# HagenMarin/SHAP-Transformer-ASR

Hardware: NVIDIA B200
Metric: masked_coalition_forwards_per_sec (higher is better)
Workload: dtype bf16

## Files before the change

### shap_transformer_asr_b200/csrc/common.cuh

```cuda
#pragma once
#include <cuda_runtime.h>
#include <cuda_bf16.h>
#include <cuda.h>
#include <stdint.h>
#include <string>

namespace w2s {

#define W2S_CUDA_OK(expr)                                                                        \
  do {                                                                                           \
    cudaError_t _e = (expr);                                                                     \
    if (_e != cudaSuccess) {                                                                     \
      return std::string(#expr) + ": " + cudaGetErrorString(_e) + " (" __FILE__ ":" +          \
             std::to_string(__LINE__) + ")";                                                     \
    }                                                                                            \
  } while (0)

}
#include <cstdlib>
#include <utility>
namespace w2s {
template <typename... KArgs, typename... Args>
inline cudaError_t launch_pdl(void (*kernel)(KArgs...), dim3 grid, dim3 block, size_t smem, cudaStream_t s, int cluster_x,
                              Args&&... args) {
// ... 178 lines not shown
      "cp.async.bulk.tensor.4d.shared::cluster.global.mbarrier::complete_tx::bytes [%0], [%1, {%3, %4, %5, %6}], [%2];"
      ::"r"(dst), "l"(reinterpret_cast<uint64_t>(map)), "r"(bar), "r"(c0), "r"(c1), "r"(c2), "r"(c3)
      : "memory");
}
__device__ __forceinline__ void tma_load_3d_mc(uint32_t dst, const CUtensorMap* map, uint32_t bar, int c0, int c1,
                                               int c2, uint16_t cta_mask) {
  asm volatile(
      "cp.async.bulk.tensor.3d.shared::cluster.global.mbarrier::complete_tx::bytes.multicast::cluster"
      " [%0], [%1, {%3, %4, %5}], [%2], %6;"
      ::"r"(dst), "l"(reinterpret_cast<uint64_t>(map)), "r"(bar), "r"(c0), "r"(c1), "r"(c2), "h"(cta_mask)
      : "memory");
}
__device__ __forceinline__ uint32_t cluster_ctarank() {
  uint32_t r;
  asm volatile("mov.u32 %0, %%cluster_ctarank;" : "=r"(r));
  return r;
}
__device__ __forceinline__ uint32_t mapa_u32(uint32_t local_addr, uint32_t rank) {
  uint32_t r;
  asm volatile("mapa.shared::cluster.u32 %0, %1, %2;" : "=r"(r) : "r"(local_addr), "r"(rank));
  return r;
}
__device__ __forceinline__ void mbar_arrive_cluster(uint32_t cluster_addr) {
  asm volatile("mbarrier.arrive.shared::cluster.b64 _, [%0];" ::"r"(cluster_addr) : "memory");
}
__device__ __forceinline__ void tma_load_3d_2sm(uint32_t dst, const CUtensorMap* map, uint32_t bar_cluster, int c0,
                                                int c1, int c2) {
  asm volatile(
      "cp.async.bulk.tensor.3d.cta_group::2.shared::cluster.global.mbarrier::complete_tx::bytes"
      " [%0], [%1, {%3, %4, %5}], [%2];"
      ::"r"(dst), "l"(reinterpret_cast<uint64_t>(map)), "r"(bar_cluster), "r"(c0), "r"(c1), "r"(c2)
      : "memory");
}
__device__ __forceinline__ void tma_load_4d_2sm(uint32_t dst, const CUtensorMap* map, uint32_t bar_cluster, int c0,
                                                int c1, int c2, int c3) {
  asm volatile(
      "cp.async.bulk.tensor.4d.cta_group::2.shared::cluster.global.mbarrier::complete_tx::bytes"
      " [%0], [%1, {%3, %4, %5, %6}], [%2];"
      ::"r"(dst), "l"(reinterpret_cast<uint64_t>(map)), "r"(bar_cluster), "r"(c0), "r"(c1), "r"(c2), "r"(c3)
      : "memory");
}
template <int kCols>
__device__ __forceinline__ void tmem_alloc_2sm(uint32_t smem_dst) {
  asm volatile("tcgen05.alloc.cta_group::2.sync.aligned.shared::cta.b32 [%0], %1;" ::"r"(smem_dst), "n"(kCols)
               : "memory");
}
__device__ __forceinline__ void tmem_relinquish_2sm() {
  asm volatile("tcgen05.relinquish_alloc_permit.cta_group::2.sync.aligned;" ::: "memory");
}
template <int kCols>
__device__ __forceinline__ void tmem_dealloc_2sm(uint32_t taddr) {
  asm volatile("tcgen05.dealloc.cta_group::2.sync.aligned.b32 %0, %1;" ::"r"(taddr), "n"(kCols) : "memory");
}
__device__ __forceinline__ void umma_bf16_2sm(uint32_t tmem_d, uint64_t desc_a, uint64_t desc_b, uint32_t idesc,
                                              uint32_t accumulate) {
  asm volatile(
      "{\n\t.reg .pred p;\n\t"
      "setp.ne.b32 p, %4, 0;\n\t"
      "tcgen05.mma.cta_group::2.kind::f16 [%0], %1, %2, %3, p;\n\t}"
      ::"r"(tmem_d), "l"(desc_a), "l"(desc_b), "r"(idesc), "r"(accumulate)
      : "memory");
}
__device__ __forceinline__ void umma_commit_2sm_mc(uint32_t bar, uint16_t cta_mask) {
  asm volatile(
      "tcgen05.commit.cta_group::2.mbarrier::arrive::one.shared::cluster.multicast::cluster.b64 [%0], %1;"
      ::"r"(bar), "h"(cta_mask)
      : "memory");
}
__device__ __forceinline__ void cluster_sync_all() {
  asm volatile("barrier.cluster.arrive.release.aligned;" ::: "memory");
  asm volatile("barrier.cluster.wait.acquire.aligned;" ::: "memory");
}
__device__ __forceinline__ void tma_store_4d(const CUtensorMap* map, uint32_t src, int c0, int c1, int c2, int c3) {
  asm volatile("cp.async.bulk.tensor.4d.global.shared::cta.bulk_group [%0, {%2, %3, %4, %5}], [%1];"
               ::"l"(reinterpret_cast<uint64_t>(map)), "r"(src), "r"(c0), "r"(c1), "r"(c2), "r"(c3)
               : "memory");
}
__device__ __forceinline__ void tma_reduce_add_4d(const CUtensorMap* map, uint32_t src, int c0, int c1, int c2, int c3) {
  asm volatile("cp.reduce.async.bulk.tensor.4d.global.shared::cta.add.tile.bulk_group [%0, {%2, %3, %4, %5}], [%1];"
               ::"l"(reinterpret_cast<uint64_t>(map)), "r"(src), "r"(c0), "r"(c1), "r"(c2), "r"(c3)
               : "memory");
}
__device__ __forceinline__ void tma_store_commit() { asm volatile("cp.async.bulk.commit_group;" ::: "memory"); }
__device__ __forceinline__ void tma_store_wait_read() { asm volatile("cp.async.bulk.wait_group.read 0;" ::: "memory"); }
__device__ __forceinline__ void tma_store_wait_all() { asm volatile("cp.async.bulk.wait_group 0;" ::: "memory"); }
__device__ __forceinline__ void sts128(uint32_t addr, uint32_t a, uint32_t b, uint32_t c, uint32_t d) {
  asm volatile("st.shared.v4.b32 [%0], {%1, %2, %3, %4};" ::"r"(addr), "r"(a), "r"(b), "r"(c), "r"(d) : "memory");
}
__device__ __forceinline__ void tma_prefetch_l2_4d(const CUtensorMap* map, int c0, int c1, int c2, int c3) {
  asm volatile("cp.async.bulk.prefetch.tensor.4d.L2.global.tile [%0, {%1, %2, %3, %4}];"
               ::"l"(reinterpret_cast<uint64_t>(map)), "r"(c0), "r"(c1), "r"(c2), "r"(c3)
               : "memory");
}
__device__ __forceinline__ void tma_prefetch_desc(const CUtensorMap* map) {
  asm volatile("prefetch.tensormap [%0];" ::"l"(reinterpret_cast<uint64_t>(map)) : "memory");
}

template <int kCols>
__device__ __forceinline__ void tmem_alloc(uint32_t smem_dst) {
  asm volatile("tcgen05.alloc.cta_group::1.sync.aligned.shared::cta.b32 [%0], %1;" ::"r"(smem_dst), "n"(kCols)
               : "memory");
}
__device__ __forceinline__ void tmem_relinquish() {
  asm volatile("tcgen05.relinquish_alloc_permit.cta_group::1.sync.aligned;" ::: "memory");
}
template <int kCols>
__device__ __forceinline__ void tmem_dealloc(uint32_t taddr) {
  asm volatile("tcgen05.dealloc.cta_group::1.sync.aligned.b32 %0, %1;" ::"r"(taddr), "n"(kCols) : "memory");
}
__device__ __forceinline__ void tc_fence_before() {
  asm volatile("tcgen05.fence::before_thread_sync;" ::: "memory");
}
__device__ __forceinline__ void tc_fence_after() {
  asm volatile("tcgen05.fence::after_thread_sync;" ::: "memory");
}
__device__ __forceinline__ void umma_bf16(uint32_t tmem_d, uint64_t desc_a, uint64_t desc_b, uint32_t idesc,
                                          uint32_t accumulate) {
  asm volatile(
      "{\n\t.reg .pred p;\n\t"
      "setp.ne.b32 p, %4, 0;\n\t"
      "tcgen05.mma.cta_group::1.kind::f16 [%0], %1, %2, %3, p;\n\t}"
      ::"r"(tmem_d), "l"(desc_a), "l"(desc_b), "r"(idesc), "r"(accumulate)
      : "memory");
}
__device__ __forceinline__ bool elect_one() {
  uint32_t pred;
  asm volatile(
      "{\n\t.reg .pred p;\n\t"
      "elect.sync _|p, 0xffffffff;\n\t"
      "selp.u32 %0, 1, 0, p;\n\t}"
      : "=r"(pred));
  return pred != 0;
}
__device__ __forceinline__ void umma_commit(uint32_t bar) {
  asm volatile("tcgen05.commit.cta_group::1.mbarrier::arrive::one.shared::cluster.b64 [%0];" ::"r"(bar)
               : "memory");
}
__device__ __forceinline__ void umma_commit_mc(uint32_t bar, uint16_t cta_mask) {
  asm volatile(
      "tcgen05.commit.cta_group::1.mbarrier::arrive::one.shared::cluster.multicast::cluster.b64 [%0], %1;"
      ::"r"(bar), "h"(cta_mask)
      : "memory");
}
__device__ __forceinline__ void tmem_ld_wait() { asm volatile("tcgen05.wait::ld.sync.aligned;" ::: "memory"); }

__device__ __forceinline__ void tmem_ld_32x32(uint32_t taddr, float (&v)[32]) {
  uint32_t r[32];
  asm volatile(
      "tcgen05.ld.sync.aligned.32x32b.x32.b32 "
      "{%0, %1, %2, %3, %4, %5, %6, %7, %8, %9, %10, %11, %12, %13, %14, %15, "
      "%16, %17, %18, %19, %20, %21, %22, %23, %24, %25, %26, %27, %28, %29, %30, %31}, [%32];"
      : "=r"(r[0]), "=r"(r[1]), "=r"(r[2]), "=r"(r[3]), "=r"(r[4]), "=r"(r[5]), "=r"(r[6]), "=r"(r[7]),
        "=r"(r[8]), "=r"(r[9]), "=r"(r[10]), "=r"(r[11]), "=r"(r[12]), "=r"(r[13]), "=r"(r[14]), "=r"(r[15]),
        "=r"(r[16]), "=r"(r[17]), "=r"(r[18]), "=r"(r[19]), "=r"(r[20]), "=r"(r[21]), "=r"(r[22]), "=r"(r[23]),
        "=r"(r[24]), "=r"(r[25]), "=r"(r[26]), "=r"(r[27]), "=r"(r[28]), "=r"(r[29]), "=r"(r[30]), "=r"(r[31])
      : "r"(taddr)
      : "memory");
  tmem_ld_wait();
#pragma unroll
  for (int i = 0; i < 32; ++i) v[i] = __uint_as_float(r[i]);
}
__device__ __forceinline__ void tmem_ld_32x32_issue(uint32_t taddr, float (&v)[32]) {
  asm volatile(
      "tcgen05.ld.sync.aligned.32x32b.x32.b32 "
      "{%0, %1, %2, %3, %4, %5, %6, %7, %8, %9, %10, %11, %12, %13, %14, %15, "
      "%16, %17, %18, %19, %20, %21, %22, %23, %24, %25, %26, %27, %28, %29, %30, %31}, [%32];"
      : "=f"(v[0]), "=f"(v[1]), "=f"(v[2]), "=f"(v[3]), "=f"(v[4]), "=f"(v[5]), "=f"(v[6]), "=f"(v[7]),
// ... 36 lines not shown
```

### shap_transformer_asr_b200/csrc/gemm.cu

```cuda
#include "gemm.cuh"
#include "gemm_epi.cuh"

#include <cudaTypedefs.h>
#include <cstdlib>
#include <mutex>

namespace w2s {

template <int BN>
struct TcCfg {
  static constexpr int BM = 128, BK = 64;
  static constexpr int A_BYTES = BM * BK * 2;
  static constexpr int B_BYTES = BN * BK * 2;
  static constexpr int STAGE_BYTES = A_BYTES + B_BYTES;
  static constexpr int STAGES = BN >= 256 ? 4 : (BN >= 128 ? 6 : 8);
  static constexpr int ACC_COLS = BN <= 32 ? 32 : (BN <= 64 ? 64 : (BN <= 128 ? 128 : 256));
  static constexpr int TMEM_COLS = 2 * ACC_COLS;
  static constexpr int CH = (BN % 32 == 0) ? 32 : 16;
  static constexpr size_t SMEM = (size_t)STAGES * STAGE_BYTES + 1024 + 256;
};

struct TileCoord {
  int g, b, m0, n0;
};
// ... 152 lines not shown
  const int nt = tile % tiles_n;
  tile /= tiles_n;
  const int mt = tile % tiles_m;
  tile /= tiles_m;
  const int b = tile % p.Bz, g = tile / p.Bz;
  const int m0 = mt * 64, n0 = nt * 64;
  const int tx = threadIdx.x & 15, ty = threadIdx.x >> 4;
  float acc[4][4] = {};
  const int rowlen = p.a_kb_per_row * 64;
  for (int k0 = 0; k0 < p.K; k0 += 16) {
    for (int i = threadIdx.x; i < 64 * 16; i += 256) {
      const int r = i >> 4, kk = i & 15;
      const int k = k0 + kk;
      float av = 0.f, wv = 0.f;
      if (k < p.K) {
        const long long row = (long long)g * p.a_g_row + m0 + r + k / rowlen;
        const long long col = (long long)g * p.a_g_col + k % rowlen;
        if (row < p.a_rows && col < p.a_cols)
          av = __bfloat162float(p.a[(long long)b * p.a_batch_stride + row * p.a_row_stride + col]);
        if (n0 + r < p.N) wv = __bfloat162float(p.w[((long long)g * p.N + n0 + r) * p.K + k]);
      }
      As[kk][r] = av;
      Ws[kk][r] = wv;
    }
    __syncthreads();
#pragma unroll
    for (int kk = 0; kk < 16; ++kk) {
      float a[4], w[4];
#pragma unroll
      for (int i = 0; i < 4; ++i) {
        a[i] = As[kk][ty * 4 + i];
        w[i] = Ws[kk][tx * 4 + i];
      }
#pragma unroll
      for (int i = 0; i < 4; ++i)
#pragma unroll
        for (int j = 0; j < 4; ++j) acc[i][j] = fmaf(a[i], w[j], acc[i][j]);
    }
    __syncthreads();
  }
#pragma unroll
  for (int i = 0; i < 4; ++i) {
    const int m = m0 + ty * 4 + i;
    if (m < p.M) epi_store<4>(p.epi, p.N, g, b, m, n0 + tx * 4, acc[i]);
  }
}

static PFN_cuTensorMapEncodeTiled_v12000 g_encode = nullptr;
static std::once_flag g_init_once;
static std::string g_init_err;

template <int BN>
static cudaError_t set_attr() {
  return cudaFuncSetAttribute(gemm_tc_kernel<BN>, cudaFuncAttributeMaxDynamicSharedMemorySize, (int)TcCfg<BN>::SMEM);
}

std::string gemm_init() {
  std::call_once(g_init_once, [] {
    void* fn = nullptr;
    cudaDriverEntryPointQueryResult qres;
    cudaError_t e = cudaGetDriverEntryPoint("cuTensorMapEncodeTiled", &fn, cudaEnableDefault, &qres);
    if (e != cudaSuccess || qres != cudaDriverEntryPointSuccess || fn == nullptr) {
      g_init_err = "cuTensorMapEncodeTiled entry point not available (driver too old?)";
      return;
    }
    g_encode = reinterpret_cast<PFN_cuTensorMapEncodeTiled_v12000>(fn);
    cudaError_t a = set_attr<256>();
    if (a == cudaSuccess) a = set_attr<128>();
    if (a == cudaSuccess) a = set_attr<64>();
    if (a == cudaSuccess) a = set_attr<48>();
    if (a == cudaSuccess) a = set_attr<32>();
    if (a != cudaSuccess) g_init_err = std::string("cudaFuncSetAttribute(gemm_tc_kernel): ") + cudaGetErrorString(a);
    if (g_init_err.empty()) g_init_err = gemm2_init();
  });
  return g_init_err;
}

std::string make_tensor_map_bf16(CUtensorMap* map, const void* base, int rank, const uint64_t* dims,
                                 const uint64_t* strides_bytes, const uint32_t* box) {
  return make_tensor_map(map, base, 0, rank, dims, strides_bytes, box);
}

std::string make_tensor_map(CUtensorMap* map, const void* base, int fp32, int rank, const uint64_t* dims,
                            const uint64_t* strides_bytes, const uint32_t* box) {
  if (!g_encode) return "tensor map encoder not initialised";
  cuuint64_t gdim[5];
  cuuint64_t gstr[5];
  cuuint32_t bx[5];
  cuuint32_t es[5];
  for (int i = 0; i < rank; ++i) {
    gdim[i] = dims[i];
    bx[i] = box[i];
    es[i] = 1;
  }
  for (int i = 0; i + 1 < rank; ++i) gstr[i] = strides_bytes[i];
  CUresult r = g_encode(map, fp32 ? CU_TENSOR_MAP_DATA_TYPE_FLOAT32 : CU_TENSOR_MAP_DATA_TYPE_BFLOAT16, rank, const_cast<void*>(base), gdim, gstr, bx, es,
                        CU_TENSOR_MAP_INTERLEAVE_NONE, CU_TENSOR_MAP_SWIZZLE_128B,
                        CU_TENSOR_MAP_L2_PROMOTION_L2_256B, CU_TENSOR_MAP_FLOAT_OOB_FILL_NONE);
  if (r != CUDA_SUCCESS) {
    std::string s = "cuTensorMapEncodeTiled failed (CUresult " + std::to_string((int)r) + ") rank=" +
                    std::to_string(rank) + " dims=";
    for (int i = 0; i < rank; ++i) s += std::to_string(dims[i]) + ",";
    s += " strides=";
    for (int i = 0; i + 1 < rank; ++i) s += std::to_string(strides_bytes[i]) + ",";
    return s;
  }
  return "";
}

static int pick_bn(int N) {
  if (N % 256 == 0) return 256;
  if (N % 128 == 0) return 128;
  if (N % 64 == 0) return 64;
  if (N % 48 == 0) return 48;
  if (N % 32 == 0) return 32;
  return 0;
}

std::string gemm_prepare(const GemmProblem& p, int num_sms, GemmLaunch* out) {
  if (p.K % 64 != 0) return "gemm: K must be a multiple of 64 (got " + std::to_string(p.K) + ")";
  const int bn = pick_bn(p.N);
  if (bn == 0) return "gemm: N must be a multiple of 32 or 48 (got " + std::to_string(p.N) + ")";
  if (p.epi.glu && (bn % 32 != 0)) return "gemm: GLU epilogue needs N % 32 == 0";
  GemmDev& d = out->dev;
  d.M = p.M; d.N = p.N; d.K = p.K; d.Bz = p.Bz; d.G = p.G;
  d.tiles_m = (p.M + 127) / 128;
  d.tiles_n = p.N / bn;
  d.num_tiles = d.tiles_m * d.tiles_n * p.Bz * p.G;
  d.num_kb = p.K / 64;
  out->mc = (bn >= 128 && d.tiles_m >= 2 && d.num_tiles >= num_sms) ? 2 : 0;
  d.units_m = out->mc ? (d.tiles_m + 1) / 2 : d.tiles_m;
  d.num_units = d.units_m * d.tiles_n * p.Bz * p.G;
  d.a_kb_per_row = p.a_kb_per_row;
  d.a_g_col = p.a_g_col;
  d.a_g_row = p.a_g_row;
  d.w_batched = p.w_batch_stride != 0;
  d.a = p.a; d.w = p.w;
  d.a_cols = p.a_cols; d.a_rows = p.a_rows; d.a_row_stride = p.a_row_stride; d.a_batch_stride = p.a_batch_stride;
  d.epi = p.epi;
  out->bn = bn;
  if (out->mc) {
    const int clusters = d.num_units < num_sms / 2 ? d.num_units : num_sms / 2;
    out->grid = 2 * clusters;
  } else {
    out->grid = d.num_units < num_sms ? d.num_units : num_sms;
  }
  out->smem = bn == 256 ? TcCfg<256>::SMEM : bn == 128 ? TcCfg<128>::SMEM : bn == 64 ? TcCfg<64>::SMEM
              : bn == 48 ? TcCfg<48>::SMEM : TcCfg<32>::SMEM;
  if ((p.a_row_stride * 2) % 16 || (p.a_batch_stride * 2) % 16 || (reinterpret_cast<uintptr_t>(p.a) % 16))
    return "gemm: A view must be 16-byte aligned in base and strides";
  {
    uint64_t dims[3] = {(uint64_t)p.a_cols, (uint64_t)p.a_rows, (uint64_t)p.a_batches};
    uint64_t str[2] = {(uint64_t)p.a_row_stride * 2, (uint64_t)(p.a_batches > 1 ? p.a_batch_stride : p.a_row_stride * p.a_rows) * 2};
    uint32_t box[3] = {64, 128, 1};
    W2S_TRY(make_tensor_map_bf16(&out->mapA, p.a, 3, dims, str, box));
  }
  {
    const uint64_t rs = (uint64_t)(p.w_row_stride ? p.w_row_stride : p.K);
    const uint64_t wr = (uint64_t)(p.w_rows ? p.w_rows : p.N);
    const uint64_t gs = (uint64_t)(p.w_g_stride ? p.w_g_stride : (long long)p.K * p.N);
    const uint64_t bs = p.w_batch_stride ? (uint64_t)p.w_batch_stride : gs * (uint64_t)p.G;
    uint64_t dims[4] = {(uint64_t)p.K, wr, (uint64_t)p.G, (uint64_t)(p.w_batch_stride ? p.Bz : 1)};
    uint64_t str[3] = {rs * 2, gs * 2, bs * 2};
    uint32_t box[4] = {64, (uint32_t)(out->mc ? bn / 2 : bn), 1, 1};
    W2S_TRY(make_tensor_map_bf16(&out->mapW, p.w, 4, dims, str, box));
  }
  out->tma_out = 0;
  if (out->mc == 2 && !p.epi.glu) {
    const uint64_t es = p.epi.out_fp32 ? 4 : 2;
    const uint64_t ldb = p.Bz > 1 ? (uint64_t)p.epi.ldb : (uint64_t)p.epi.ldm * p.M;
    const uint64_t ldg = p.G > 1 ? (uint64_t)p.epi.ldg : ldb * p.Bz;
    uint64_t dims[4] = {(uint64_t)p.N, (uint64_t)p.M, (uint64_t)p.Bz, (uint64_t)p.G};
    uint64_t str[3] = {(uint64_t)p.epi.ldm * es, ldb * es, ldg * es};
    uint32_t box[4] = {p.epi.out_fp32 ? 32u : 64u, 32, 1, 1};
    if (str[0] % 16 == 0 && str[1] % 16 == 0 && str[2] % 16 == 0 && reinterpret_cast<uintptr_t>(p.epi.out) % 16 == 0) {
      W2S_TRY(make_tensor_map(&out->mapOut, p.epi.out, p.epi.out_fp32, 4, dims, str, box));
      out->tma_out = 1;
    }
  }
  return "";
}

std::string gemm_launch_tc(const GemmLaunch& l, cudaStream_t s) {
  if (l.mc == 2) return gemm2_launch(l, s);
  switch (l.bn) {
    case 256: W2S_CUDA_OK(launch_pdl(gemm_tc_kernel<256>, dim3(l.grid), dim3(384), l.smem, s, 1, l.mapA, l.mapW, l.dev)); break;
    case 128: W2S_CUDA_OK(launch_pdl(gemm_tc_kernel<128>, dim3(l.grid), dim3(384), l.smem, s, 1, l.mapA, l.mapW, l.dev)); break;
    case 64: W2S_CUDA_OK(launch_pdl(gemm_tc_kernel<64>, dim3(l.grid), dim3(384), l.smem, s, 1, l.mapA, l.mapW, l.dev)); break;
    case 48: W2S_CUDA_OK(launch_pdl(gemm_tc_kernel<48>, dim3(l.grid), dim3(384), l.smem, s, 1, l.mapA, l.mapW, l.dev)); break;
    case 32: W2S_CUDA_OK(launch_pdl(gemm_tc_kernel<32>, dim3(l.grid), dim3(384), l.smem, s, 1, l.mapA, l.mapW, l.dev)); break;
    default: return "gemm: bad BN";
  }
  W2S_CUDA_OK(cudaGetLastError());
  return "";
}

std::string gemm_launch_simt(const GemmLaunch& l, cudaStream_t s) {
  const GemmDev& d = l.dev;
  const long long tiles = (long long)((d.M + 63) / 64) * ((d.N + 63) / 64) * d.Bz * d.G;
  gemm_simt_kernel<<<(unsigned)tiles, 256, 0, s>>>(d);
  W2S_CUDA_OK(cudaGetLastError());
  return "";
}

}
```

### shap_transformer_asr_b200/csrc/gemm.cuh

```cuda
#pragma once
#include "common.cuh"

namespace w2s {

struct EpiParams {
  const float* bias = nullptr;
  int act = ACT_NONE;
  int glu = 0;
  float alpha = 1.0f;
  const void* residual = nullptr;
  int res_fp32 = 0;
  void* out = nullptr;
  int out_fp32 = 0;
  long long ldg = 0, ldb = 0, ldm = 0;
};

struct GemmProblem {
  const __nv_bfloat16* a = nullptr;
  long long a_cols = 0, a_rows = 0, a_batches = 1;
  long long a_row_stride = 0, a_batch_stride = 0;
  int a_kb_per_row = 1, a_g_col = 0, a_g_row = 0;
  const __nv_bfloat16* w = nullptr;
  long long w_row_stride = 0, w_g_stride = 0, w_batch_stride = 0;
  int w_rows = 0;
  int M = 0, N = 0, K = 0, Bz = 1, G = 1;
  EpiParams epi;
};

struct GemmDev {
  int M, N, K, Bz, G;
  int tiles_m, tiles_n, num_tiles, num_kb;
  int units_m, num_units;
  int a_kb_per_row, a_g_col, a_g_row;
  int w_batched;
  const __nv_bfloat16* a;
  const __nv_bfloat16* w;
  long long a_cols, a_rows, a_row_stride, a_batch_stride;
  EpiParams epi;
};

struct GemmLaunch {
  CUtensorMap mapA, mapW;
  CUtensorMap mapOut;
  int tma_out = 0;
  GemmDev dev;
  int bn = 0;
  int mc = 0;
  int grid = 0;
  size_t smem = 0;
};

std::string gemm_prepare(const GemmProblem& p, int num_sms, GemmLaunch* out);
std::string gemm_launch_tc(const GemmLaunch& l, cudaStream_t s);
std::string gemm_launch_simt(const GemmLaunch& l, cudaStream_t s);
std::string gemm2_init();
std::string gemm2_launch(const GemmLaunch& l, cudaStream_t s);
std::string gemm_init();

std::string make_tensor_map_bf16(CUtensorMap* map, const void* base, int rank, const uint64_t* dims,
                                 const uint64_t* strides_bytes, const uint32_t* box);
std::string make_tensor_map(CUtensorMap* map, const void* base, int fp32, int rank, const uint64_t* dims,
                            const uint64_t* strides_bytes, const uint32_t* box);

}
```

### shap_transformer_asr_b200/csrc/gemm2.cu

```cuda
#include "gemm.cuh"
#include "gemm_epi.cuh"

namespace w2s {

template <int BN>
struct Tc2Cfg {
  static constexpr int A_BYTES = 128 * 64 * 2;
  static constexpr int B_BYTES = (BN / 2) * 64 * 2;
  static constexpr int STAGE_BYTES = A_BYTES + B_BYTES;
  static constexpr int EPI_BYTES = 8 * 4096 + 8 * 512;
  static constexpr int STAGES = (227 * 1024 - 1024 - 256 - EPI_BYTES) / STAGE_BYTES > 8
                                    ? 8 : (227 * 1024 - 1024 - 256 - EPI_BYTES) / STAGE_BYTES;
  static constexpr int ACC_COLS = BN;
  static constexpr int TMEM_COLS = 2 * ACC_COLS;
  static constexpr size_t SMEM = (size_t)STAGES * STAGE_BYTES + EPI_BYTES + 1024 + 256;
};

template <int BN>
__global__ void __launch_bounds__(384, 1)
gemm_tc2_kernel(const __grid_constant__ CUtensorMap mapA, const __grid_constant__ CUtensorMap mapW,
                const __grid_constant__ CUtensorMap mapOut, const GemmDev p, const int tma_out) {
  using C = Tc2Cfg<BN>;
  const uint32_t rank = cluster_ctarank();
  const bool leader = rank == 0;
  const int unit0 = (int)(blockIdx.x >> 1), unit_step = (int)(gridDim.x >> 1);
  extern __shared__ uint8_t smem_raw[];
  const uint32_t raw = smem_u32(smem_raw);
  const uint32_t tiles = (raw + 1023u) & ~1023u;
  uint8_t* tiles_ptr = smem_raw + (tiles - raw);
  const uint32_t epi_smem = tiles + C::STAGES * C::STAGE_BYTES;
  const uint32_t bars = epi_smem + C::EPI_BYTES;
  auto full_bar = [&](int s) { return bars + 8u * s; };
  auto empty_bar = [&](int s) { return bars + 8u * (C::STAGES + s); };
  auto tfull_bar = [&](int a) { return bars + 8u * (2 * C::STAGES + a); };
  auto tempty_bar = [&](int a) { return bars + 8u * (2 * C::STAGES + 2 + a); };
  const uint32_t tmem_slot = bars + 8u * (2 * C::STAGES + 4);
  volatile uint32_t* tmem_slot_ptr =
      reinterpret_cast<volatile uint32_t*>(tiles_ptr + C::STAGES * C::STAGE_BYTES + C::EPI_BYTES + 8 * (2 * C::STAGES + 4));

  const int warp = threadIdx.x >> 5, lane = threadIdx.x & 31;
  if (warp == 8 && lane == 0) {
    tma_prefetch_desc(&mapA);
    tma_prefetch_desc(&mapW);
    if (tma_out) tma_prefetch_desc(&mapOut);
  }
  if (warp == 9 && lane == 0) {
    for (int s = 0; s < C::STAGES; ++s) {
      mbar_init(full_bar(s), 1);
      mbar_init(empty_bar(s), 1);
    }
    for (int a = 0; a < 2; ++a) {
      mbar_init(tfull_bar(a), 1);
      mbar_init(tempty_bar(a), 16);
    }
    fence_barrier_init();
    fence_proxy_async();
  }
  if (warp == 10) {
    tmem_alloc_2sm<C::TMEM_COLS>(tmem_slot);
    tmem_relinquish_2sm();
  }
  tc_fence_before();
  __syncthreads();
  cluster_sync_all();
  tc_fence_after();
  const uint32_t tmem_base = *tmem_slot_ptr;

  if (warp == 8) {
    if (elect_one()) {
      int stage = 0;
      uint32_t phase = 0;
      for (int unit = unit0; unit < p.num_units; unit += unit_step) {
        int nt = unit % p.tiles_n;
        int r = unit / p.tiles_n;
        const int mu = r % p.units_m;
        r /= p.units_m;
        const int b = r % p.Bz, g = r / p.Bz;
        const int m0 = (2 * mu + (int)rank) * 128, n0 = nt * BN;
        for (int kb = 0; kb < p.num_kb; ++kb) {
          mbar_wait(empty_bar(stage), phase ^ 1u);
          const uint32_t full_leader = mapa_u32(full_bar(stage), 0);
          if (leader) mbar_expect_tx(full_bar(stage), 2 * C::STAGE_BYTES);
          const int krow = kb / p.a_kb_per_row;
          const int kcol = kb - krow * p.a_kb_per_row;
          const uint32_t sa = tiles + stage * C::STAGE_BYTES;
          tma_load_3d_2sm(sa, &mapA, full_leader, g * p.a_g_col + kcol * 64, g * p.a_g_row + m0 + krow, b);
          tma_load_4d_2sm(sa + C::A_BYTES, &mapW, full_leader, kb * 64, n0 + (int)rank * (BN / 2), g, p.w_batched ? b : 0);
          if (++stage == C::STAGES) {
            stage = 0;
            phase ^= 1u;
          }
        }
      }
    }
  } else if (warp == 9) {
    if (leader && elect_one()) {
      constexpr uint32_t idesc = umma_idesc_bf16(256, BN);
      int stage = 0;
      uint32_t phase = 0;
      int acc = 0;
      uint32_t acc_phase = 0;
      for (int unit = unit0; unit < p.num_units; unit += unit_step) {
        mbar_wait(tempty_bar(acc), acc_phase ^ 1u);
        tc_fence_after();
        const uint32_t d_tmem = tmem_base + acc * C::ACC_COLS;
        for (int kb = 0; kb < p.num_kb; ++kb) {
          mbar_wait(full_bar(stage), phase);
          tc_fence_after();
          const uint32_t sa = tiles + stage * C::STAGE_BYTES;
          const uint64_t da = umma_desc_sw128(sa);
          const uint64_t db = umma_desc_sw128(sa + C::A_BYTES);
#pragma unroll
          for (int k = 0; k < 4; ++k) umma_bf16_2sm(d_tmem, da + 2u * k, db + 2u * k, idesc, (kb | k) != 0 ? 1u : 0u);
          umma_commit_2sm_mc(empty_bar(stage), (uint16_t)0x3);
          if (++stage == C::STAGES) {
            stage = 0;
            phase ^= 1u;
          }
        }
        umma_commit_2sm_mc(tfull_bar(acc), (uint16_t)0x3);
        acc ^= 1;
        if (acc == 0) acc_phase ^= 1u;
      }
    }
  } else if (warp < 8) {
    const int q = warp & 3, hsel = warp >> 2;
    const bool lead = elect_one();
    const uint32_t stg = epi_smem + warp * 4096;
    const uint32_t stg_row = stg + lane * 128;
    float* sbias = reinterpret_cast<float*>(tiles_ptr + C::STAGES * C::STAGE_BYTES + 8 * 4096 + warp * 512);
    const bool f32 = p.epi.out_fp32 != 0;
    const bool reduce_add = tma_out && f32 && p.epi.res_fp32 && p.epi.residual == p.epi.out;
    int acc = 0;
    uint32_t acc_phase = 0;
    for (int unit = unit0; unit < p.num_units; unit += unit_step) {
      int nt = unit % p.tiles_n;
      int r = unit / p.tiles_n;
      const int mu = r % p.units_m;
      r /= p.units_m;
      const int b = r % p.Bz, g = r / p.Bz;
      const int m0 = (2 * mu + (int)rank) * 128, n0 = nt * BN;
      const int m = m0 + q * 32 + lane;
      const bool row_ok = m < p.M;
      const uint32_t t0 = tmem_base + (static_cast<uint32_t>(q * 32) << 16) + acc * C::ACC_COLS;
      if (tma_out) {
        const int bw = f32 ? 32 : 64;
        const int nblk = BN / (2 * bw);
        if (p.epi.bias) {
          for (int i = lane; i < nblk * bw; i += 32) {
            const int col = (2 * (i / bw) + hsel) * bw + (i % bw);
            sbias[i] = __ldg(p.epi.bias + (long long)g * p.N + n0 + col);
          }
        }
        __syncwarp();
        mbar_wait(tfull_bar(acc), acc_phase);
        tc_fence_after();
        const int nsub = f32 ? nblk : 2 * nblk;
        auto sub_col = [&](int sidx) { return f32 ? (2 * sidx + hsel) * 32 : (2 * (sidx >> 1) + hsel) * 64 + (sidx & 1) * 32; };
        float v[32];
        tmem_ld_32x32_issue(t0 + sub_col(0), v);
#pragma unroll 1
        for (int sidx = 0; sidx < nsub; ++sidx) {
          const int c = sub_col(sidx);
          const int sub = f32 ? 0 : (sidx & 1);
          tmem_ld_wait();
          epi_math32(p.epi, p.epi.bias ? sbias + sidx * 32 : nullptr, p.N, g, b, m, n0 + c, row_ok, v, reduce_add);
          if (f32) {
            if (lead) tma_store_wait_read();
            __syncwarp();
#pragma unroll
            for (int j = 0; j < 8; ++j)
              sts128(stg_row + (((uint32_t)j ^ ((uint32_t)lane & 7u)) << 4), __float_as_uint(v[4 * j]),
                     __float_as_uint(v[4 * j + 1]), __float_as_uint(v[4 * j + 2]), __float_as_uint(v[4 * j + 3]));
            if (sidx + 1 < nsub) tmem_ld_32x32_issue(t0 + sub_col(sidx + 1), v);
          } else {
            uint32_t pk[16];
#pragma unroll
            for (int j = 0; j < 16; ++j) pk[j] = pack_bf16x2(v[2 * j], v[2 * j + 1]);
            if (sidx + 1 < nsub) tmem_ld_32x32_issue(t0 + sub_col(sidx + 1), v);
            if (sub == 0) {
              if (lead) tma_store_wait_read();
              __syncwarp();
            }
#pragma unroll
            for (int j = 0; j < 4; ++j)
              sts128(stg_row + (((uint32_t)(sub * 4 + j) ^ ((uint32_t)lane & 7u)) << 4), pk[4 * j], pk[4 * j + 1],
                     pk[4 * j + 2], pk[4 * j + 3]);
          }
          if (f32 || sub == 1) {
            const int cblk = f32 ? c : c - 32;
            fence_proxy_async();
            __syncwarp();
            if (lead) {
              if (reduce_add) tma_reduce_add_4d(&mapOut, stg, n0 + cblk, m0 + q * 32, b, g);
              else tma_store_4d(&mapOut, stg, n0 + cblk, m0 + q * 32, b, g);
              tma_store_commit();
            }
          }
        }
      } else {
        mbar_wait(tfull_bar(acc), acc_phase);
        tc_fence_after();
#pragma unroll 1
        for (int c = hsel * 32; c < BN; c += 64) {
          float v[32];
          tmem_ld_32x32(t0 + c, v);
          if (row_ok) epi_store<32>(p.epi, p.N, g, b, m, n0 + c, v);
        }
      }
      tc_fence_before();
      __syncwarp();
      if (lane == 0) {
        if (leader) mbar_arrive(tempty_bar(acc));
        else mbar_arrive_cluster(mapa_u32(tempty_bar(acc), 0));
      }
      acc ^= 1;
      if (acc == 0) acc_phase ^= 1u;
    }
    if (tma_out && lead) tma_store_wait_all();
  }

  tc_fence_before();
  __syncthreads();
  cluster_sync_all();
  if (warp == 10) {
    tc_fence_after();
    tmem_dealloc_2sm<C::TMEM_COLS>(tmem_base);
  }
}

std::string gemm2_init() {
  cudaError_t e = cudaFuncSetAttribute(gemm_tc2_kernel<256>, cudaFuncAttributeMaxDynamicSharedMemorySize,
                                       (int)Tc2Cfg<256>::SMEM);
  if (e == cudaSuccess)
    e = cudaFuncSetAttribute(gemm_tc2_kernel<128>, cudaFuncAttributeMaxDynamicSharedMemorySize, (int)Tc2Cfg<128>::SMEM);
  if (e != cudaSuccess) return std::string("cudaFuncSetAttribute(gemm_tc2_kernel): ") + cudaGetErrorString(e);
  return "";
}

size_t gemm2_smem(int bn) { return bn == 256 ? Tc2Cfg<256>::SMEM : Tc2Cfg<128>::SMEM; }

template <int BN>
static cudaError_t launch2(const GemmLaunch& l, cudaStream_t s) {
  return launch_pdl(gemm_tc2_kernel<BN>, dim3(l.grid), dim3(384), Tc2Cfg<BN>::SMEM, s, 2, l.mapA, l.mapW,
                    l.tma_out ? l.mapOut : l.mapA, l.dev, l.tma_out);
}

std::string gemm2_launch(const GemmLaunch& l, cudaStream_t s) {
  if (l.bn == 256) W2S_CUDA_OK(launch2<256>(l, s));
  else if (l.bn == 128) W2S_CUDA_OK(launch2<128>(l, s));
  else return "gemm (CTA pair): BN must be 256 or 128";
  return "";
}

}
```

### shap_transformer_asr_b200/csrc/gemm_epi.cuh

```cuda
#pragma once
#include "gemm.cuh"

namespace w2s {

template <int CH>
__device__ __forceinline__ void epi_store(const EpiParams& e, int N, int g, int b, int m, int ncol0, float* v) {
  if (ncol0 >= N) return;
  if (e.bias) {
    const float4* bp = reinterpret_cast<const float4*>(e.bias + (long long)g * N + ncol0);
#pragma unroll
    for (int j = 0; j < CH / 4; ++j) {
      const float4 t = __ldg(bp + j);
      v[4 * j] += t.x;
      v[4 * j + 1] += t.y;
      v[4 * j + 2] += t.z;
      v[4 * j + 3] += t.w;
    }
  }
  if (e.act == ACT_GELU) {
#pragma unroll
    for (int j = 0; j < CH; j += 2) {
      const float2 r = gelu_erf2(make_float2(v[j], v[j + 1]));
      v[j] = r.x;
      v[j + 1] = r.y;
    }
  } else if (e.act == ACT_SWISH) {
#pragma unroll
    for (int j = 0; j < CH; ++j) v[j] = swish(v[j]);
  }
  int nout0 = ncol0, nvals = CH, Nout = N;
  if (e.glu) {
#pragma unroll
    for (int j = 0; j < CH / 2; ++j) v[j] = v[2 * j] * rcp_approx(1.0f + ex2_approx(-1.4426950408889634f * v[2 * j + 1]));
    nout0 = ncol0 >> 1;
    nvals = CH / 2;
    Nout = N >> 1;
  }
  const long long off = (long long)g * e.ldg + (long long)b * e.ldb + (long long)m * e.ldm + nout0;
  if constexpr (CH < 8) {
#pragma unroll
    for (int j = 0; j < CH; ++j) {
      if (j < nvals && nout0 + j < Nout) {
        float r = 0.f;
        if (e.residual)
          r = e.res_fp32 ? reinterpret_cast<const float*>(e.residual)[off + j]
                         : __bfloat162float(reinterpret_cast<const __nv_bfloat16*>(e.residual)[off + j]);
        const float o = fmaf(v[j], e.alpha, r);
        if (e.out_fp32) reinterpret_cast<float*>(e.out)[off + j] = o;
        else reinterpret_cast<__nv_bfloat16*>(e.out)[off + j] = __float2bfloat16_rn(o);
      }
    }
  } else {
    if (e.residual) {
      if (e.res_fp32) {
        const float* rp = reinterpret_cast<const float*>(e.residual) + off;
#pragma unroll
        for (int j = 0; j < CH; j += 4) {
          if (j < nvals && nout0 + j < Nout) {
            float4 r = *reinterpret_cast<const float4*>(rp + j);
            v[j] = fmaf(v[j], e.alpha, r.x);
            v[j + 1] = fmaf(v[j + 1], e.alpha, r.y);
            v[j + 2] = fmaf(v[j + 2], e.alpha, r.z);
            v[j + 3] = fmaf(v[j + 3], e.alpha, r.w);
          }
        }
      } else {
        const __nv_bfloat16* rp = reinterpret_cast<const __nv_bfloat16*>(e.residual) + off;
#pragma unroll
        for (int j = 0; j < CH; j += 4) {
          if (j < nvals && nout0 + j < Nout) {
            uint2 r = *reinterpret_cast<const uint2*>(rp + j);
            v[j] = fmaf(v[j], e.alpha, bf16_lo(r.x));
            v[j + 1] = fmaf(v[j + 1], e.alpha, bf16_hi(r.x));
            v[j + 2] = fmaf(v[j + 2], e.alpha, bf16_lo(r.y));
            v[j + 3] = fmaf(v[j + 3], e.alpha, bf16_hi(r.y));
          }
        }
      }
    } else if (e.alpha != 1.0f) {
#pragma unroll
      for (int j = 0; j < CH; ++j) v[j] *= e.alpha;
    }
    if (e.out_fp32) {
      float* op = reinterpret_cast<float*>(e.out) + off;
#pragma unroll
      for (int j = 0; j < CH; j += 4)
        if (j < nvals && nout0 + j < Nout)
          *reinterpret_cast<float4*>(op + j) = make_float4(v[j], v[j + 1], v[j + 2], v[j + 3]);
    } else {
      __nv_bfloat16* op = reinterpret_cast<__nv_bfloat16*>(e.out) + off;
#pragma unroll
      for (int j = 0; j < CH; j += 8) {
        if (j < nvals && nout0 + j < Nout) {
          uint4 u;
          u.x = pack_bf16x2(v[j], v[j + 1]);
          u.y = pack_bf16x2(v[j + 2], v[j + 3]);
          u.z = pack_bf16x2(v[j + 4], v[j + 5]);
          u.w = pack_bf16x2(v[j + 6], v[j + 7]);
          *reinterpret_cast<uint4*>(op + j) = u;
        }
      }
    }
  }
}


__device__ __forceinline__ void epi_math32(const EpiParams& e, const float* sbias, int N, int g, int b, int m,
                                           int ncol0, bool row_ok, float* v, bool skip_residual = false) {
  if (sbias) {
#pragma unroll
    for (int j = 0; j < 8; ++j) {
      const float4 t = *reinterpret_cast<const float4*>(sbias + 4 * j);
      v[4 * j] += t.x;
      v[4 * j + 1] += t.y;
      v[4 * j + 2] += t.z;
      v[4 * j + 3] += t.w;
    }
  }
  if (e.act == ACT_GELU) {
#pragma unroll
    for (int j = 0; j < 32; j += 2) {
      const float2 r = gelu_erf2(make_float2(v[j], v[j + 1]));
      v[j] = r.x;
      v[j + 1] = r.y;
    }
  } else if (e.act == ACT_SWISH) {
#pragma unroll
    for (int j = 0; j < 32; ++j) v[j] = swish(v[j]);
  }
  if (e.residual && !skip_residual) {
    if (row_ok) {
      const long long off = (long long)g * e.ldg + (long long)b * e.ldb + (long long)m * e.ldm + ncol0;
      if (e.res_fp32) {
        const float* rp = reinterpret_cast<const float*>(e.residual) + off;
#pragma unroll
        for (int j = 0; j < 32; j += 4) {
          const float4 r = *reinterpret_cast<const float4*>(rp + j);
          v[j] = fmaf(v[j], e.alpha, r.x);
          v[j + 1] = fmaf(v[j + 1], e.alpha, r.y);
          v[j + 2] = fmaf(v[j + 2], e.alpha, r.z);
          v[j + 3] = fmaf(v[j + 3], e.alpha, r.w);
        }
      } else {
        const __nv_bfloat16* rp = reinterpret_cast<const __nv_bfloat16*>(e.residual) + off;
#pragma unroll
        for (int j = 0; j < 32; j += 8) {
          const uint4 r = *reinterpret_cast<const uint4*>(rp + j);
          v[j] = fmaf(v[j], e.alpha, bf16_lo(r.x));
          v[j + 1] = fmaf(v[j + 1], e.alpha, bf16_hi(r.x));
          v[j + 2] = fmaf(v[j + 2], e.alpha, bf16_lo(r.y));
          v[j + 3] = fmaf(v[j + 3], e.alpha, bf16_hi(r.y));
          v[j + 4] = fmaf(v[j + 4], e.alpha, bf16_lo(r.z));
          v[j + 5] = fmaf(v[j + 5], e.alpha, bf16_hi(r.z));
          v[j + 6] = fmaf(v[j + 6], e.alpha, bf16_lo(r.w));
          v[j + 7] = fmaf(v[j + 7], e.alpha, bf16_hi(r.w));
        }
      }
    }
  } else if (e.alpha != 1.0f) {
#pragma unroll
    for (int j = 0; j < 32; ++j) v[j] *= e.alpha;
  }
}

}
```

Measured before the change: 12490.

## Restructure CTA-pair GEMM epilogue with 16 warps, smaller swizzled TMA boxes, early TMEM release

Templates the pair GEMM kernel on the number of epilogue warps and picks 16 epilogue warps for activation-heavy, short-K GEMMs. Output TMA stores now use 32-column (bf16) or 16-column (fp32) boxes with 64B swizzle, and several store buffers are kept in flight by waiting on all but the newest groups. Bias for the next tile is prefetched into registers, and the accumulator is released to the MMA warp before the final epilogue math runs. The aim is to hide epilogue cost behind the mainloop; the risks are more TMA store instructions, higher register pressure and a more complex sync pattern.

```diff
diff --git a/shap_transformer_asr_b200/csrc/common.cuh b/shap_transformer_asr_b200/csrc/common.cuh
--- a/shap_transformer_asr_b200/csrc/common.cuh
+++ b/shap_transformer_asr_b200/csrc/common.cuh
@@ -284,7 +284,10 @@
                : "memory");
 }
 __device__ __forceinline__ void tma_store_commit() { asm volatile("cp.async.bulk.commit_group;" ::: "memory"); }
-__device__ __forceinline__ void tma_store_wait_read() { asm volatile("cp.async.bulk.wait_group.read 0;" ::: "memory"); }
+template <int kPending = 0>
+__device__ __forceinline__ void tma_store_wait_read() {
+  asm volatile("cp.async.bulk.wait_group.read %0;" ::"n"(kPending) : "memory");
+}
 __device__ __forceinline__ void tma_store_wait_all() { asm volatile("cp.async.bulk.wait_group 0;" ::: "memory"); }
 __device__ __forceinline__ void sts128(uint32_t addr, uint32_t a, uint32_t b, uint32_t c, uint32_t d) {
   asm volatile("st.shared.v4.b32 [%0], {%1, %2, %3, %4};" ::"r"(addr), "r"(a), "r"(b), "r"(c), "r"(d) : "memory");
diff --git a/shap_transformer_asr_b200/csrc/gemm.cu b/shap_transformer_asr_b200/csrc/gemm.cu
--- a/shap_transformer_asr_b200/csrc/gemm.cu
+++ b/shap_transformer_asr_b200/csrc/gemm.cu
@@ -258,8 +258,9 @@
 }
 
 std::string make_tensor_map(CUtensorMap* map, const void* base, int fp32, int rank, const uint64_t* dims,
-                            const uint64_t* strides_bytes, const uint32_t* box) {
+                            const uint64_t* strides_bytes, const uint32_t* box, int swizzle_bytes) {
   if (!g_encode) return "tensor map encoder not initialised";
+  if (swizzle_bytes != 128 && swizzle_bytes != 64) return "make_tensor_map: swizzle must be 64 or 128 B";
   cuuint64_t gdim[5];
   cuuint64_t gstr[5];
   cuuint32_t bx[5];
@@ -271,7 +272,8 @@
   }
   for (int i = 0; i + 1 < rank; ++i) gstr[i] = strides_bytes[i];
   CUresult r = g_encode(map, fp32 ? CU_TENSOR_MAP_DATA_TYPE_FLOAT32 : CU_TENSOR_MAP_DATA_TYPE_BFLOAT16, rank, const_cast<void*>(base), gdim, gstr, bx, es,
-                        CU_TENSOR_MAP_INTERLEAVE_NONE, CU_TENSOR_MAP_SWIZZLE_128B,
+                        CU_TENSOR_MAP_INTERLEAVE_NONE,
+                        swizzle_bytes == 64 ? CU_TENSOR_MAP_SWIZZLE_64B : CU_TENSOR_MAP_SWIZZLE_128B,
                         CU_TENSOR_MAP_L2_PROMOTION_L2_256B, CU_TENSOR_MAP_FLOAT_OOB_FILL_NONE);
   if (r != CUDA_SUCCESS) {
     std::string s = "cuTensorMapEncodeTiled failed (CUresult " + std::to_string((int)r) + ") rank=" +
@@ -348,9 +350,9 @@
     const uint64_t ldg = p.G > 1 ? (uint64_t)p.epi.ldg : ldb * p.Bz;
     uint64_t dims[4] = {(uint64_t)p.N, (uint64_t)p.M, (uint64_t)p.Bz, (uint64_t)p.G};
     uint64_t str[3] = {(uint64_t)p.epi.ldm * es, ldb * es, ldg * es};
-    uint32_t box[4] = {p.epi.out_fp32 ? 32u : 64u, 32, 1, 1};
+    uint32_t box[4] = {p.epi.out_fp32 ? 16u : 32u, 32, 1, 1};
     if (str[0] % 16 == 0 && str[1] % 16 == 0 && str[2] % 16 == 0 && reinterpret_cast<uintptr_t>(p.epi.out) % 16 == 0) {
-      W2S_TRY(make_tensor_map(&out->mapOut, p.epi.out, p.epi.out_fp32, 4, dims, str, box));
+      W2S_TRY(make_tensor_map(&out->mapOut, p.epi.out, p.epi.out_fp32, 4, dims, str, box, 64));
       out->tma_out = 1;
     }
   }
diff --git a/shap_transformer_asr_b200/csrc/gemm.cuh b/shap_transformer_asr_b200/csrc/gemm.cuh
--- a/shap_transformer_asr_b200/csrc/gemm.cuh
+++ b/shap_transformer_asr_b200/csrc/gemm.cuh
@@ -60,6 +60,6 @@
 std::string make_tensor_map_bf16(CUtensorMap* map, const void* base, int rank, const uint64_t* dims,
                                  const uint64_t* strides_bytes, const uint32_t* box);
 std::string make_tensor_map(CUtensorMap* map, const void* base, int fp32, int rank, const uint64_t* dims,
-                            const uint64_t* strides_bytes, const uint32_t* box);
+                            const uint64_t* strides_bytes, const uint32_t* box, int swizzle_bytes = 128);
 
 }
diff --git a/shap_transformer_asr_b200/csrc/gemm2.cu b/shap_transformer_asr_b200/csrc/gemm2.cu
--- a/shap_transformer_asr_b200/csrc/gemm2.cu
+++ b/shap_transformer_asr_b200/csrc/gemm2.cu
@@ -3,12 +3,15 @@
 
 namespace w2s {
 
-template <int BN>
+template <int BN, int EW>
 struct Tc2Cfg {
   static constexpr int A_BYTES = 128 * 64 * 2;
   static constexpr int B_BYTES = (BN / 2) * 64 * 2;
   static constexpr int STAGE_BYTES = A_BYTES + B_BYTES;
-  static constexpr int EPI_BYTES = 8 * 4096 + 8 * 512;
+  static constexpr int EPI_WARPS = EW;
+  static constexpr int BOXES = 16 / EW;
+  static constexpr int BIAS_BYTES = 4096 / EW;
+  static constexpr int EPI_BYTES = 32768 + 4096;
   static constexpr int STAGES = (227 * 1024 - 1024 - 256 - EPI_BYTES) / STAGE_BYTES > 8
                                     ? 8 : (227 * 1024 - 1024 - 256 - EPI_BYTES) / STAGE_BYTES;
   static constexpr int ACC_COLS = BN;
@@ -16,11 +19,11 @@
   static constexpr size_t SMEM = (size_t)STAGES * STAGE_BYTES + EPI_BYTES + 1024 + 256;
 };
 
-template <int BN>
-__global__ void __launch_bounds__(384, 1)
+template <int BN, int EW>
+__global__ void __launch_bounds__(EW * 32 + 64, 1)
 gemm_tc2_kernel(const __grid_constant__ CUtensorMap mapA, const __grid_constant__ CUtensorMap mapW,
                 const __grid_constant__ CUtensorMap mapOut, const GemmDev p, const int tma_out) {
-  using C = Tc2Cfg<BN>;
+  using C = Tc2Cfg<BN, EW>;
   const uint32_t rank = cluster_ctarank();
   const bool leader = rank == 0;
   const int unit0 = (int)(blockIdx.x >> 1), unit_step = (int)(gridDim.x >> 1);
@@ -39,24 +42,24 @@
       reinterpret_cast<volatile uint32_t*>(tiles_ptr + C::STAGES * C::STAGE_BYTES + C::EPI_BYTES + 8 * (2 * C::STAGES + 4));
 
   const int warp = threadIdx.x >> 5, lane = threadIdx.x & 31;
-  if (warp == 8 && lane == 0) {
+  if (warp == EW && lane == 0) {
     tma_prefetch_desc(&mapA);
     tma_prefetch_desc(&mapW);
     if (tma_out) tma_prefetch_desc(&mapOut);
   }
-  if (warp == 9 && lane == 0) {
+  if (warp == EW + 1 && lane == 0) {
     for (int s = 0; s < C::STAGES; ++s) {
       mbar_init(full_bar(s), 1);
       mbar_init(empty_bar(s), 1);
     }
     for (int a = 0; a < 2; ++a) {
       mbar_init(tfull_bar(a), 1);
-      mbar_init(tempty_bar(a), 16);
+      mbar_init(tempty_bar(a), 2 * C::EPI_WARPS);
     }
     fence_barrier_init();
     fence_proxy_async();
   }
-  if (warp == 10) {
+  if (warp == EW) {
     tmem_alloc_2sm<C::TMEM_COLS>(tmem_slot);
     tmem_relinquish_2sm();
   }
@@ -66,7 +69,7 @@
   tc_fence_after();
   const uint32_t tmem_base = *tmem_slot_ptr;
 
-  if (warp == 8) {
+  if (warp == EW) {
     if (elect_one()) {
       int stage = 0;
       uint32_t phase = 0;
@@ -93,7 +96,7 @@
         }
       }
     }
-  } else if (warp == 9) {
+  } else if (warp == EW + 1) {
     if (leader && elect_one()) {
       constexpr uint32_t idesc = umma_idesc_bf16(256, BN);
       int stage = 0;
@@ -123,96 +126,114 @@
         if (acc == 0) acc_phase ^= 1u;
       }
     }
-  } else if (warp < 8) {
-    const int q = warp & 3, hsel = warp >> 2;
+  } else if (warp < C::EPI_WARPS) {
+    constexpr int NQ = EW / 4;
+    const int q = warp & 3, grp = warp >> 2;
     const bool lead = elect_one();
-    const uint32_t stg = epi_smem + warp * 4096;
-    const uint32_t stg_row = stg + lane * 128;
-    float* sbias = reinterpret_cast<float*>(tiles_ptr + C::STAGES * C::STAGE_BYTES + 8 * 4096 + warp * 512);
+    const uint32_t stg0 = epi_smem + warp * (C::BOXES * 2048);
+    float* sbias = reinterpret_cast<float*>(tiles_ptr + C::STAGES * C::STAGE_BYTES + 32768 + warp * C::BIAS_BYTES);
     const bool f32 = p.epi.out_fp32 != 0;
     const bool reduce_add = tma_out && f32 && p.epi.res_fp32 && p.epi.residual == p.epi.out;
+    const int bw = f32 ? 16 : 32;
+    const int nsub = BN / (NQ * bw);
+    auto sub_col = [&](int sidx) { return (NQ * sidx + grp) * bw; };
+    auto decode = [&](int unit, int& nt, int& mu, int& b, int& g) {
+      nt = unit % p.tiles_n;
+      int r = unit / p.tiles_n;
+      mu = r % p.units_m;
+      r /= p.units_m;
+      b = r % p.Bz;
+      g = r / p.Bz;
+    };
+    constexpr int NB = BN / (32 * NQ);
+    float bnext[NB];
+    auto load_bias = [&](int unit) {
+      int nt, mu, b, g;
+      decode(unit, nt, mu, b, g);
+      const float* bp = p.epi.bias + (long long)g * p.N + nt * BN;
+#pragma unroll
+      for (int k = 0; k < NB; ++k) {
+        const int i = lane + 32 * k;
+        bnext[k] = __ldg(bp + sub_col(i / bw) + (i % bw));
+      }
+    };
+    const bool tma_bias = tma_out && p.epi.bias;
+    if (tma_bias && unit0 < p.num_units) load_bias(unit0);
     int acc = 0;
     uint32_t acc_phase = 0;
     for (int unit = unit0; unit < p.num_units; unit += unit_step) {
-      int nt = unit % p.tiles_n;
-      int r = unit / p.tiles_n;
-      const int mu = r % p.units_m;
-      r /= p.units_m;
-      const int b = r % p.Bz, g = r / p.Bz;
+      int nt, mu, b, g;
+      decode(unit, nt, mu, b, g);
       const int m0 = (2 * mu + (int)rank) * 128, n0 = nt * BN;
       const int m = m0 + q * 32 + lane;
       const bool row_ok = m < p.M;
       const uint32_t t0 = tmem_base + (static_cast<uint32_t>(q * 32) << 16) + acc * C::ACC_COLS;
+      auto release_acc = [&]() {
+        tc_fence_before();
+        __syncwarp();
+        if (lane == 0) {
+          if (leader) mbar_arrive(tempty_bar(acc));
+          else mbar_arrive_cluster(mapa_u32(tempty_bar(acc), 0));
+        }
+      };
       if (tma_out) {
-        const int bw = f32 ? 32 : 64;
-        const int nblk = BN / (2 * bw);
-        if (p.epi.bias) {
-          for (int i = lane; i < nblk * bw; i += 32) {
-            const int col = (2 * (i / bw) + hsel) * bw + (i % bw);
-            sbias[i] = __ldg(p.epi.bias + (long long)g * p.N + n0 + col);
-          }
-        }
-        __syncwarp();
+        if (tma_bias) {
+          __syncwarp();
+#pragma unroll
+          for (int k = 0; k < NB; ++k) sbias[lane + 32 * k] = bnext[k];
+          if (unit + unit_step < p.num_units) load_bias(unit + unit_step);
+          __syncwarp();
+        }
         mbar_wait(tfull_bar(acc), acc_phase);
         tc_fence_after();
-        const int nsub = f32 ? nblk : 2 * nblk;
-        auto sub_col = [&](int sidx) { return f32 ? (2 * sidx + hsel) * 32 : (2 * (sidx >> 1) + hsel) * 64 + (sidx & 1) * 32; };
-        float v[32];
-        tmem_ld_32x32_issue(t0 + sub_col(0), v);
 #pragma unroll 1
         for (int sidx = 0; sidx < nsub; ++sidx) {
           const int c = sub_col(sidx);
-          const int sub = f32 ? 0 : (sidx & 1);
-          tmem_ld_wait();
-          epi_math32(p.epi, p.epi.bias ? sbias + sidx * 32 : nullptr, p.N, g, b, m, n0 + c, row_ok, v, reduce_add);
+          const uint32_t stg = stg0 + (uint32_t)(sidx % C::BOXES) * 2048u;
+          const float* sb = p.epi.bias ? sbias + sidx * bw : nullptr;
+          auto chunk = [&](int j) { return stg + lane * 64 + (((uint32_t)j ^ (((uint32_t)lane >> 1) & 3u)) << 4); };
           if (f32) {
-            if (lead) tma_store_wait_read();
+            float v[16];
+            tmem_ld_32x16(t0 + c, v);
+            if (sidx + 1 == nsub) release_acc();
+            epi_math<16>(p.epi, sb, p.N, g, b, m, n0 + c, row_ok, v, reduce_add);
+            if (lead) tma_store_wait_read<C::BOXES - 1>();
             __syncwarp();
 #pragma unroll
-            for (int j = 0; j < 8; ++j)
-              sts128(stg_row + (((uint32_t)j ^ ((uint32_t)lane & 7u)) << 4), __float_as_uint(v[4 * j]),
-                     __float_as_uint(v[4 * j + 1]), __float_as_uint(v[4 * j + 2]), __float_as_uint(v[4 * j + 3]));
-            if (sidx + 1 < nsub) tmem_ld_32x32_issue(t0 + sub_col(sidx + 1), v);
+            for (int j = 0; j < 4; ++j)
+              sts128(chunk(j), __float_as_uint(v[4 * j]), __float_as_uint(v[4 * j + 1]), __float_as_uint(v[4 * j + 2]),
+                     __float_as_uint(v[4 * j + 3]));
           } else {
+            float v[32];
+            tmem_ld_32x32(t0 + c, v);
+            if (sidx + 1 == nsub) release_acc();
+            epi_math<32>(p.epi, sb, p.N, g, b, m, n0 + c, row_ok, v, reduce_add);
             uint32_t pk[16];
 #pragma unroll
             for (int j = 0; j < 16; ++j) pk[j] = pack_bf16x2(v[2 * j], v[2 * j + 1]);
-            if (sidx + 1 < nsub) tmem_ld_32x32_issue(t0 + sub_col(sidx + 1), v);
-            if (sub == 0) {
-              if (lead) tma_store_wait_read();
-              __syncwarp();
-            }
-#pragma unroll
-            for (int j = 0; j < 4; ++j)
-              sts128(stg_row + (((uint32_t)(sub * 4 + j) ^ ((uint32_t)lane & 7u)) << 4), pk[4 * j], pk[4 * j + 1],
-                     pk[4 * j + 2], pk[4 * j + 3]);
-          }
-          if (f32 || sub == 1) {
-            const int cblk = f32 ? c : c - 32;
-            fence_proxy_async();
+            if (lead) tma_store_wait_read<C::BOXES - 1>();
             __syncwarp();
-            if (lead) {
-              if (reduce_add) tma_reduce_add_4d(&mapOut, stg, n0 + cblk, m0 + q * 32, b, g);
-              else tma_store_4d(&mapOut, stg, n0 + cblk, m0 + q * 32, b, g);
-              tma_store_commit();
-            }
+#pragma unroll
+            for (int j = 0; j < 4; ++j) sts128(chunk(j), pk[4 * j], pk[4 * j + 1], pk[4 * j + 2], pk[4 * j + 3]);
+          }
+          fence_proxy_async();
+          __syncwarp();
+          if (lead) {
+            if (reduce_add) tma_reduce_add_4d(&mapOut, stg, n0 + c, m0 + q * 32, b, g);
+            else tma_store_4d(&mapOut, stg, n0 + c, m0 + q * 32, b, g);
+            tma_store_commit();
           }
         }
       } else {
         mbar_wait(tfull_bar(acc), acc_phase);
         tc_fence_after();
 #pragma unroll 1
-        for (int c = hsel * 32; c < BN; c += 64) {
+        for (int c = grp * 32; c < BN; c += 32 * NQ) {
           float v[32];
           tmem_ld_32x32(t0 + c, v);
           if (row_ok) epi_store<32>(p.epi, p.N, g, b, m, n0 + c, v);
         }
-      }
-      tc_fence_before();
-      __syncwarp();
-      if (lane == 0) {
-        if (leader) mbar_arrive(tempty_bar(acc));
-        else mbar_arrive_cluster(mapa_u32(tempty_bar(acc), 0));
+        release_acc();
       }
       acc ^= 1;
       if (acc == 0) acc_phase ^= 1u;
@@ -223,32 +244,39 @@
   tc_fence_before();
   __syncthreads();
   cluster_sync_all();
-  if (warp == 10) {
+  if (warp == EW) {
     tc_fence_after();
     tmem_dealloc_2sm<C::TMEM_COLS>(tmem_base);
   }
 }
 
+template <int BN, int EW>
+static cudaError_t set_attr2() {
+  return cudaFuncSetAttribute(gemm_tc2_kernel<BN, EW>, cudaFuncAttributeMaxDynamicSharedMemorySize,
+                              (int)Tc2Cfg<BN, EW>::SMEM);
+}
+
 std::string gemm2_init() {
-  cudaError_t e = cudaFuncSetAttribute(gemm_tc2_kernel<256>, cudaFuncAttributeMaxDynamicSharedMemorySize,
-                                       (int)Tc2Cfg<256>::SMEM);
-  if (e == cudaSuccess)
-    e = cudaFuncSetAttribute(gemm_tc2_kernel<128>, cudaFuncAttributeMaxDynamicSharedMemorySize, (int)Tc2Cfg<128>::SMEM);
+  cudaError_t e = set_attr2<256, 8>();
+  if (e == cudaSuccess) e = set_attr2<256, 16>();
+  if (e == cudaSuccess) e = set_attr2<128, 8>();
+  if (e == cudaSuccess) e = set_attr2<128, 16>();
   if (e != cudaSuccess) return std::string("cudaFuncSetAttribute(gemm_tc2_kernel): ") + cudaGetErrorString(e);
   return "";
 }
 
-size_t gemm2_smem(int bn) { return bn == 256 ? Tc2Cfg<256>::SMEM : Tc2Cfg<128>::SMEM; }
-
-template <int BN>
+size_t gemm2_smem(int bn) { return bn == 256 ? Tc2Cfg<256, 8>::SMEM : Tc2Cfg<128, 8>::SMEM; }
+
+template <int BN, int EW>
 static cudaError_t launch2(const GemmLaunch& l, cudaStream_t s) {
-  return launch_pdl(gemm_tc2_kernel<BN>, dim3(l.grid), dim3(384), Tc2Cfg<BN>::SMEM, s, 2, l.mapA, l.mapW,
-                    l.tma_out ? l.mapOut : l.mapA, l.dev, l.tma_out);
+  return launch_pdl(gemm_tc2_kernel<BN, EW>, dim3(l.grid), dim3(EW * 32 + 64), Tc2Cfg<BN, EW>::SMEM, s, 2, l.mapA,
+                    l.mapW, l.tma_out ? l.mapOut : l.mapA, l.dev, l.tma_out);
 }
 
 std::string gemm2_launch(const GemmLaunch& l, cudaStream_t s) {
-  if (l.bn == 256) W2S_CUDA_OK(launch2<256>(l, s));
-  else if (l.bn == 128) W2S_CUDA_OK(launch2<128>(l, s));
+  const bool epi_heavy = l.dev.epi.act != ACT_NONE && l.dev.num_kb <= 16;
+  if (l.bn == 256) W2S_CUDA_OK((epi_heavy ? launch2<256, 16>(l, s) : launch2<256, 8>(l, s)));
+  else if (l.bn == 128) W2S_CUDA_OK((epi_heavy ? launch2<128, 16>(l, s) : launch2<128, 8>(l, s)));
   else return "gemm (CTA pair): BN must be 256 or 128";
   return "";
 }
diff --git a/shap_transformer_asr_b200/csrc/gemm_epi.cuh b/shap_transformer_asr_b200/csrc/gemm_epi.cuh
--- a/shap_transformer_asr_b200/csrc/gemm_epi.cuh
+++ b/shap_transformer_asr_b200/csrc/gemm_epi.cuh
@@ -105,11 +105,12 @@
 }
 
 
-__device__ __forceinline__ void epi_math32(const EpiParams& e, const float* sbias, int N, int g, int b, int m,
-                                           int ncol0, bool row_ok, float* v, bool skip_residual = false) {
+template <int CH>
+__device__ __forceinline__ void epi_math(const EpiParams& e, const float* sbias, int N, int g, int b, int m,
+                                         int ncol0, bool row_ok, float* v, bool skip_residual = false) {
   if (sbias) {
 #pragma unroll
-    for (int j = 0; j < 8; ++j) {
+    for (int j = 0; j < CH / 4; ++j) {
       const float4 t = *reinterpret_cast<const float4*>(sbias + 4 * j);
       v[4 * j] += t.x;
       v[4 * j + 1] += t.y;
@@ -119,14 +120,14 @@
   }
   if (e.act == ACT_GELU) {
 #pragma unroll
-    for (int j = 0; j < 32; j += 2) {
+    for (int j = 0; j < CH; j += 2) {
       const float2 r = gelu_erf2(make_float2(v[j], v[j + 1]));
       v[j] = r.x;
       v[j + 1] = r.y;
     }
   } else if (e.act == ACT_SWISH) {
 #pragma unroll
-    for (int j = 0; j < 32; ++j) v[j] = swish(v[j]);
+    for (int j = 0; j < CH; ++j) v[j] = swish(v[j]);
   }
   if (e.residual && !skip_residual) {
     if (row_ok) {
@@ -134,7 +135,7 @@
       if (e.res_fp32) {
         const float* rp = reinterpret_cast<const float*>(e.residual) + off;
 #pragma unroll
-        for (int j = 0; j < 32; j += 4) {
+        for (int j = 0; j < CH; j += 4) {
           const float4 r = *reinterpret_cast<const float4*>(rp + j);
           v[j] = fmaf(v[j], e.alpha, r.x);
           v[j + 1] = fmaf(v[j + 1], e.alpha, r.y);
@@ -144,7 +145,7 @@
       } else {
         const __nv_bfloat16* rp = reinterpret_cast<const __nv_bfloat16*>(e.residual) + off;
 #pragma unroll
-        for (int j = 0; j < 32; j += 8) {
+        for (int j = 0; j < CH; j += 8) {
           const uint4 r = *reinterpret_cast<const uint4*>(rp + j);
           v[j] = fmaf(v[j], e.alpha, bf16_lo(r.x));
           v[j + 1] = fmaf(v[j + 1], e.alpha, bf16_hi(r.x));
@@ -159,7 +160,7 @@
     }
   } else if (e.alpha != 1.0f) {
 #pragma unroll
-    for (int j = 0; j < 32; ++j) v[j] *= e.alpha;
+    for (int j = 0; j < CH; ++j) v[j] *= e.alpha;
   }
 }
 
```

Result: no change. 12520, median of 6 (+0.3%).
